# riveSunder/therldaisyworld

Measured on AMD Instinct MI355X. Metric: cell-updates/sec (grid x batch), fused stencil+growth step, higher is better.
Workload: dtype f32

## Files before the change

### therldaisyworld_amd/csrc/dw_api.hip

```cpp
#include <hip/hip_runtime.h>

#include <cmath>
#include <cstdarg>
#include <cstdio>
#include <cstdlib>
#include <cstring>
#include <memory>
#include <new>
#include <optional>
#include <type_traits>
#include <vector>

#include "../../include/daisyworld_hip.h"
#include "dw_kernels.hpp"
#include "dw_host_util.hpp"
#include "dw_plan.hpp"
#include "dw_series.hpp"
#include "dw_episode_staging.hpp"

using namespace dw;

static thread_local char g_err[512] = "";

static int fail(int code, const char* fmt, ...) {
// ... 31 lines not shown
struct PinnedMem {
    static int alloc(void** p, size_t n) { return hipHostMalloc(p, n, hipHostMallocDefault); }
    static int release(void* p) { return hipHostFree(p); }
};
template <class T> using DevBuf = Buf<T, DeviceMem>;
template <class T> using PinnedBuf = Buf<T, PinnedMem>;

struct dw_handle {
    dw_params prm;
    hipStream_t stream = nullptr;
    bool own_stream = false;
    size_t cells = 0;
    DevBuf<plane_t> L16[2];
    DevBuf<plane_t> D16[2];
    int cur = 0;
    DevBuf<double> L64;
    DevBuf<double> D64;
    DevBuf<float> U32L;
    DevBuf<float> U32D;
    UnqKind unq_kind = UNQ_F64;
    UnqOwner unq = OWN_NONE;
    bool have_state = false;
    bool stepped = false;
    double L_last = 0.0;
    bool L_per_world = false;
    bool P_per_world = false;
    DevBuf<int> idx;
    DevBuf<double> st;
    DevBuf<int> action;
    DevBuf<int> action_tmp;
// ... 93 lines not shown

struct SyncOnExit {
    hipStream_t stream;
    bool armed = true;
    explicit SyncOnExit(hipStream_t s) : stream(s) {}
    ~SyncOnExit() { if (armed) (void)hipStreamSynchronize(stream); }
    void disarm() { armed = false; }
};

static int alloc_failed(int rc, const char* what, size_t bytes) {
    (void)hipGetLastError();
    const hipError_t e = static_cast<hipError_t>(rc);
    return fail(e == hipErrorOutOfMemory ? DW_ENOMEM : DW_EHIP, "allocating %s (%zu bytes) failed: %s", what, bytes,
                hipGetErrorString(e));
}
template <class B>
static int reserve(B& buf, const char* what, size_t need, size_t first_size = 0) {
    const int rc = buf.reserve(need, first_size);
    return rc ? alloc_failed(rc, what, need) : DW_OK;
}

static int alloc_group(dw_handle* h, const char* what, std::initializer_list<GroupItem<DeviceMem>> group) {
    static int fail_left = -1;
    if (h->created && fail_left < 0)
        if (const char* e = test_hook("DW_TEST_FAIL_GROUP_ALLOC")) fail_left = std::atoi(e);
    const bool armed = h->created && fail_left > 0;
    if (armed) t_fail_in = (int)group.size();
    const int rc = dw::alloc_group(group);
    if (armed && t_fail_in == 0) --fail_left;
    t_fail_in = 0;
    size_t bytes = 0;
    for (const auto& g : group) bytes += g.bytes;
    return rc ? alloc_failed(rc, what, bytes) : DW_OK;
}

static void release_unquantised(dw_handle* h) {
    if (h->unq != OWN_NONE || !h->U32L.get()) return;
    for (const auto& sn : h->snap)
        if (sn.valid && sn.unq == OWN_PREV) return;
    if (h->cells * 2 * sizeof(float) < ((size_t)1 << 30)) return;
    (void)hipStreamSynchronize(h->stream);
    h->U32L.reset();
    h->U32D.reset();
}

static void drop_unquantised_previous(dw_handle* h) {
    if (h->unq == OWN_PREV) { h->unq = OWN_NONE; h->stepped = false; }
    release_unquantised(h);
}

static int ensure_u32(dw_handle* h) {
    const size_t n = sizeof(float) * h->cells;
    return alloc_group(h, "two float32 planes", {{h->U32L, n}, {h->U32D, n}});
}

static int ensure_f64(dw_handle* h) {
    const size_t n = sizeof(double) * h->cells;
    return alloc_group(h, "two float64 planes", {{h->L64, n}, {h->D64, n}});
}

static int run_episode_impl(dw_handle* h, int32_t nsteps, const double* L_schedule, int policy_mode,
                            const uint8_t* use_table, const int8_t* table, uint32_t threshold_k,
                            uint8_t* world_alive, uint8_t* agent_ok, dw_world_stats* trace = nullptr,
                            dw_temp_stats* temps = nullptr);
static bool episode_kernel_applies(const dw_handle* h);
enum EpisodeForm { EPISODE_STEPWISE, EPISODE_WORKGROUP, EPISODE_WAVE };
static EpisodeForm episode_form(const dw_handle* h);
static EpisodeForm episode_mlp_form(const dw_handle* h, size_t* lds_bytes = nullptr);
static int worlds_per_block(int cells) { return cells <= 256 ? 4 : (cells <= 1024 ? 2 : 1); }
static int observe_into_scratch(dw_handle* h, double L_init, size_t extra_bytes, bool reward_tail = false);

static int ensure_scratch(dw_handle* h, size_t bytes) { return reserve(h->scratch, "scratch", bytes); }

static int ensure_ep_buf(dw_handle* h, size_t bytes) {
    return reserve(h->ep_buf, "the episode staging buffer", bytes, (size_t)4 << 20);
}

struct EpisodeBuffers {
    using R = EpisodeStaging;
    dw_handle* h;
    const EpisodeStaging S;
    unsigned char* img = nullptr;
    std::vector<PhysF32> p32_own;
    std::vector<unsigned char> ut_own;

    EpisodeBuffers(dw_handle* h_, const EpisodeStaging& S_) : h(h_), S(S_) {}
    bool out_direct = false;
    int alloc(bool staged, bool inputs_only = false) {
        if (int rc = ensure_ep_buf(h, S.total)) return rc;
        if (!staged) return DW_OK;
        const size_t image = inputs_only ? S.off[R::WORLD_ALIVE] : S.total;
        if (int rc = reserve(h->ep_pinned, "the page-locked episode staging", image, (size_t)1 << 20)) return rc;
        img = h->ep_pinned.get();
        out_direct = inputs_only;
        return DW_OK;
    }
    template <class T = unsigned char>
    T* dev(R::Region r) const { return S.at<T>(h->ep_buf.get(), r); }
    PhysF32* p32() {
        if (img) return S.at<PhysF32>(img, R::P32);
        p32_own.resize(S.bytes[R::P32] / sizeof(PhysF32));
        return p32_own.data();
    }
    int upload(const double* Ls, size_t n_ls, bool first, const uint8_t* use_table, const int8_t* table) {
        const bool have_table = table && S.bn;
        const size_t ut_bytes = S.bytes[R::USE_TABLE];
        auto to_dev = [&](R::Region r, const void* src, size_t bytes) {
// ... 204 lines not shown
        FixQ fq;
        fq.entries = h->fixq.get();
        fq.counts = reinterpret_cast<unsigned int*>(o.stats + p.batch + 1);
        fq.qcap = h->qcap;
        fq.redo_tiles = h->redo_tiles.get();
        auto tiled = [&](auto TCQ, auto RPT) {
            return with_bool(ex, [&](auto EX) { return launch_tiled<TCQ, RPT, EX>(h, iL, iD, o, fq); });
        };
        if (pl.tcq == 64) return with_int<8, 4, 2>(pl.rpt, [&](auto RPT) { return tiled(int_c<64>{}, RPT); });
        return pl.tcq == 32 ? tiled(int_c<32>{}, int_c<4>{}) : tiled(int_c<16>{}, int_c<2>{});
    }
    HIPCHK(hipGetLastError());
    return DW_OK;
}

static void step_done(dw_handle* h, double L, bool stepped, bool per_world = false, bool per_world_constants = false) {
    h->cur = 1 - h->cur;
    h->sp = 1 - h->sp;
    h->unq = h->unq == OWN_CUR ? OWN_PREV : OWN_NONE;
    h->stepped = stepped;
    h->L_last = L;
    h->L_per_world = per_world;
    h->P_per_world = per_world && per_world_constants;
    release_unquantised(h);
}

static void episode_done(dw_handle* h, double L_last, bool per_world) {
    h->unq = OWN_NONE;
    h->stepped = true;
    h->L_last = per_world ? 0.0 : L_last;
    h->L_per_world = per_world;
    h->P_per_world = per_world;
// ... 312 lines not shown
            });
        });
    } else {
        with_bool(pstats != nullptr, [&](auto STATS) {
            with_fused_layout(pl, [&](auto MODE, auto PACK) {
                hipLaunchKernelGGL((step_stream_fused2<MODE, PACK, STATS>), grid, dim3(256), 0, h->stream, inL, inD, o.L, o.D, g,
                                   P1, P2, o.zero_me, o.zero_n, pstats, thr_hi);
            });
        });
    }
    HIPCHK(hipGetLastError());
    step_done(h, L2, false);
    return DW_OK;
}

static int launch_agents(dw_handle* h, const int* d_action, int act_b, int act_n, bool standalone = false,
                         double* d_reward = nullptr, unsigned char* d_done = nullptr, unsigned char* d_ok = nullptr) {
    const dw_params& p = h->prm;
    if (p.n_agents == 0) return DW_OK;
    NEED(h->have_state, DW_ESTATE, "no state uploaded");
    NEED(h->have_agents, DW_ESTATE, "no agents uploaded (call dw_upload_agents or dw_init_random)");
    NEED(p.collision_mode == 0 || standalone, DW_EINVAL,
         "collision_mode=1: call dw_update_agents, apply the collision pass (it consumes the caller's RNG) to the "
         "downloaded agent states, upload them, then dw_step without actions");
    const int blocks = (p.batch + 63) / 64;
    with_planes(h, h->unq == OWN_CUR, h->cur, [&](auto* L, auto* D) {
        using T = elem_t<decltype(L)>;
        hipLaunchKernelGGL(agents_update<T>, dim3(blocks), dim3(64), 0, h->stream, L, D, h->idx.get(), h->st.get(), d_action,
                           act_b, act_n, p.batch, p.n_agents, p.height, p.width, p.agent_gamma,
                           p.collision_mode == 0 ? 1 : 0, d_reward, d_done, d_ok);
// ... 491 lines not shown
        HIPCHK(hipEventRecord(h->evf0, h->stream));
        int launched = 0;
        while (nsteps - s0 >= 3) {
            const double L1 = L;
            advance();
            const double L2 = L;
            advance();
            int rc = launch_forward_fused2(h, L1, L2);
            if (rc) return rc;
            s0 += 2;
            launched += 1;
        }
        HIPCHK(hipEventRecord(h->evf1, h->stream));
        h->fused_launches = launched;
    }
    for (int s = s0; s < nsteps; ++s) {
        int rc;
        if (use_device_actions) {
            rc = launch_agents(h, h->action.get(), h->prm.batch, h->prm.n_agents);
            if (rc) return rc;
        }
        rc = launch_forward(h, L);
        if (rc) return rc;
        advance();
    }
    *L_io = L;
    return DW_OK;
}

static bool ensemble_pairs(const dw_handle* h) { return h->plan.trace_pairs && h->prm.precision == DW_PRECISION_FAST; }
// ... 13 lines not shown
}

struct PwTable {
    dw_handle* h;
    const PwLayout lay;
    hipEvent_t uploaded = nullptr;
    bool in_flight = false;
    PwTable(dw_handle* h_, const PwLayout& lay_) : h(h_), lay(lay_) {}
    PwTable(const PwTable&) = delete;
    ~PwTable() { if (uploaded) (void)hipEventDestroy(uploaded); }
    unsigned char* img() const { return h->pw_pinned.get(); }
    unsigned char* dev() const { return h->pw_tab.get(); }
    GroupItem<DeviceMem> item() const { return {h->pw_tab, lay.bytes}; }
    int alloc(const char* what, std::initializer_list<GroupItem<DeviceMem>> group) {
        if (int rc = alloc_group(h, what, group)) return rc;
        if (int rc = reserve(h->pw_pinned, "the page-locked image of the per-world constants", lay.bytes)) {
            h->pw_tab.reset();
            return rc;
        }
        HIPCHK(hipEventCreateWithFlags(&uploaded, hipEventDisableTiming));
        return DW_OK;
    }
    int next_chunk(const SeriesSchedule& q, size_t c, const double* Ls, WorldRows& worlds, bool first_bound = false) {
        if (in_flight) HIPCHK(hipEventSynchronize(uploaded));
        fill_chunk(q, c, Ls, worlds, lay, img());
        if (first_bound) worlds.first_bound(Ls, lay.p32(img(), 0), h->unq_kind == UNQ_F64, h->sw.first_slack, lay.fb(img()));
        auto part = [&](size_t off, size_t bytes) { return hipMemcpyAsync(dev() + off, img() + off, bytes, hipMemcpyHostToDevice, h->stream); };
        const size_t singles = q.chunks[c].singles, pairs = q.chunks[c].pairs;
        if (singles) {
            HIPCHK(part(0, sizeof(PhysF32) * singles * lay.B));
            HIPCHK(part(lay.o64, sizeof(PhysF64) * singles * lay.B));
// ... 318 lines not shown
    HIPCHK(hipMemcpyAsync(obs, h->scratch.get(), sizeof(double) * bn * 63, hipMemcpyDeviceToHost, h->stream));
    HIPCHK(hipStreamSynchronize(h->stream));
    return DW_OK;
}

int dw_env_step(dw_handle* h, const int32_t* action, int32_t action_b, int32_t action_n, double L, double* obs,
                double* reward, uint8_t* done) {
    NEED(h, DW_EINVAL, "null handle");
    const dw_params& p = h->prm;
    HIPCHK(hipSetDevice(p.device));
    const size_t bn = (size_t)p.batch * p.n_agents;
    auto up = [](size_t v) { return (v + 255) / 256 * 256; };
    const bool big_obs = sizeof(double) * bn * 63 > ((size_t)512 << 10);
    const size_t o_act = 0, o_obs = up(sizeof(int) * bn), o_rew = o_obs + sizeof(double) * bn * 63;
    const size_t total = up(o_rew + sizeof(double) * bn + bn) + 256;
    if (int rc = reserve(h->pinned, "the page-locked step staging", total)) return rc;
    if (action) {
        NEED(action_b >= 0 && action_n >= 0 && action_b <= p.batch && action_n <= p.n_agents, DW_EINVAL,
             "action block %dx%d exceeds (B,N)=(%d,%d)", action_b, action_n, p.batch, p.n_agents);
        const size_t na = (size_t)action_b * action_n;
        if (na) {
            std::memcpy(h->pinned.get() + o_act, action, sizeof(int) * na);
            HIPCHK(hipMemcpyAsync(h->action_tmp.get(), h->pinned.get() + o_act, sizeof(int) * na, hipMemcpyHostToDevice, h->stream));
        }
        int rc = launch_agents(h, h->action_tmp.get(), action_b, action_n);
        if (rc) return rc;
    }
    int rc = launch_forward(h, L);
    if (rc) return rc;
    if (bn) {
        NEED(h->have_agents, DW_ESTATE, "no agents");
// ... 178 lines not shown
    NEED(n_members == 1 || (member_a && member_b), DW_EINVAL, "several parameter sets need both member maps");
    NEED_SHARED_L(h, "the episode's first observation");
    const size_t wbytes = sizeof(double) * 1808 * (size_t)n_members;
    EpisodeRegions regions;
    regions.rows = K; regions.mlp = true; regions.trace = records; regions.temps = temps != nullptr;
    const EpisodeStaging S(K, (size_t)B, (size_t)N, regions);
    using R = EpisodeStaging;
    const size_t o_ma = S.off[R::MEMBER_A], o_mb = S.off[R::MEMBER_B], o_p32 = S.off[R::P32], o_ls = S.off[R::LS];
    if (temps)
        if (int rc = alloc_group(h, "the temperature reduction", {{h->temp_part, temp_part_bytes(h)}})) return rc;
    if (int erc = ensure_ep_buf(h, S.total)) return erc;
    if (params) {
        if (h->mlp_members != n_members) {
            h->mlp_w.reset();
            h->mlp_members = 0;
            if (int rc = reserve(h->mlp_w, "the parameter sets", wbytes)) return rc;
            h->mlp_members = n_members;
        }
    }
    const double* d_w = h->mlp_w.get();
    const int* d_ma = member_a ? reinterpret_cast<const int*>(h->ep_buf.get() + o_ma) : nullptr;
    const int* d_mb = member_b ? reinterpret_cast<const int*>(h->ep_buf.get() + o_mb) : nullptr;
    double* d_r = S.at<double>(h->ep_buf.get(), R::REWARD);
    unsigned char* d_d = S.at<unsigned char>(h->ep_buf.get(), R::DONE);
    StatsDev* const d_rows = S.at<StatsDev>(h->ep_buf.get(), R::TRACE);
    TempStatsDev* const d_trows = reinterpret_cast<TempStatsDev*>(h->ep_buf.get() + S.temps_off());
    SyncOnExit guard(h->stream);
    if (params) HIPCHK(hipMemcpyAsync(h->mlp_w.get(), params, wbytes, hipMemcpyHostToDevice, h->stream));
    if (member_a) HIPCHK(hipMemcpyAsync(h->ep_buf.get() + o_ma, member_a, sizeof(int) * B, hipMemcpyHostToDevice, h->stream));
    if (member_b) HIPCHK(hipMemcpyAsync(h->ep_buf.get() + o_mb, member_b, sizeof(int) * B, hipMemcpyHostToDevice, h->stream));
    const int Cc = p.height * p.width;
// ... 750 lines not shown
                 g.chunk * 8);
        if (pl.allow_fuse) {
            const size_t n = std::strlen(buf);
            snprintf(buf + n, buflen - n, "; dw_step_n fuses step pairs (step_stream_fused2%s%s",
                     p.precision == DW_PRECISION_EXACT ? "_exact" : "",
                     pl.seam_strips ? "_seam_pw, format buffer accesses" : (pl.fmt_planes ? "_fmt_pw, format buffer accesses" : ""));
            if (pl.seam_strips) {
                const size_t m = std::strlen(buf);
                snprintf(buf + m, buflen - m, ", seam strips: %d x %d columns + %d columns of %d row bands per wave", pl.seam_geom.ncs,
                         kSeamCols, pl.left_geom.cols_per_strip, pl.left_geom.wpr);
            }
            if (pl.row_landing) {
                const size_t m = std::strlen(buf);
                snprintf(buf + m, buflen - m, ", rows land in place: step_stream_fused2_land_seam_pw + _land_left_pw");
            }
            const size_t m = std::strlen(buf);
            snprintf(buf + m, buflen - m, ")");
        }
    } else if (pl.kind == STEP_TILED) {
        const int TR = (256 / pl.tcq) * pl.rpt;
        snprintf(buf, buflen,
                 "step_tiled<TCQ=%d,RPT=%d,%s> tile=%dx%d cells, %zu B LDS/workgroup, %d tiles, grid=%d x 256 threads, "
                 "XCD-chunked",
                 pl.tcq, pl.rpt, prec, TR, pl.tcq * 4, pl.tile_lds, pl.geom.ntiles, pl.geom.chunk * 8);
    } else {
        snprintf(buf, buflen, "step_generic<%s> one thread per cell, grid=(%d,%d) x 256 threads", prec,
                 (p.height * p.width + 255) / 256, p.batch);
    }
    {
        const size_t n = std::strlen(buf);
// ... 92 lines not shown
```

### therldaisyworld_amd/csrc/dw_host_util.hpp

```cpp
#pragma once
#include <cstddef>
#include <initializer_list>

namespace dw {

template <class Policy>
class Block {
public:
    Block() = default;
    Block(const Block&) = delete;
    Block& operator=(const Block&) = delete;
    Block(Block&& o) noexcept : p_(o.p_), bytes_(o.bytes_) { o.p_ = nullptr; o.bytes_ = 0; }
    Block& operator=(Block&& o) noexcept {
        if (this != &o) {
            reset();
            p_ = o.p_; bytes_ = o.bytes_;
            o.p_ = nullptr; o.bytes_ = 0;
        }
        return *this;
    }
    ~Block() { reset(); }

    void* raw() const { return p_; }
    size_t bytes() const { return bytes_; }
// ... 17 lines not shown
        bytes_ = bytes;
        return 0;
    }

private:
    void* p_ = nullptr;
    size_t bytes_ = 0;
};

template <class T, class Policy>
class Buf : public Block<Policy> {
public:
    T* get() const { return static_cast<T*>(this->raw()); }
};

template <class Policy>
struct GroupItem {
    Block<Policy>& owner;
    size_t bytes;
};

template <class Policy>
int alloc_group(std::initializer_list<GroupItem<Policy>> group) {
    bool held = true;
    for (const auto& g : group) held = held && g.owner.bytes() >= g.bytes;
    if (held) return 0;
    for (const auto& g : group) g.owner.reset();
    for (const auto& g : group) {
        if (const int rc = g.owner.take(g.bytes)) {
            for (const auto& r : group) r.owner.reset();
// ... 8 lines not shown
```

### therldaisyworld_amd/csrc/dw_plan.hpp

```cpp
#pragma once
#include <climits>
#include <cmath>
#include <cstddef>
#include <cstdio>
#include <cstdlib>
#include <cstring>

#include "../../include/daisyworld_hip.h"
#include "dw_types.hpp"

namespace dw {

struct Switches {
    bool no_sym = false, no_pack = false, no_fuse = false, no_ring = false, no_fmt_planes = false, no_seam_strips = false,
         no_row_landing = false,
         no_episode_kernel = false,
         no_episode_wave = false, no_agent_fuse = false, no_agent_preapply = false, first_f64 = false,
         first_generic = false, force_rescan = false, test_hooks = false;
    int pack_min_strips = -1, strip_rows = 0, tile_rpt = 0, queue_cap = -1, mismatch_cap = -1, trace_rows = 0, frame_ring = 0;
    double first_slack = -1.0;
    char kernel[16] = {0};
    char text[256] = {0};
};
inline const char* test_hook(const char* name) {
    return std::getenv("DW_TEST_HOOKS") ? std::getenv(name) : nullptr;
}
inline Switches read_switches() {
    Switches w;
    auto note = [&](const char* name, const char* val) {
        const size_t n = std::strlen(w.text);
        snprintf(w.text + n, sizeof(w.text) - n, "%s%s%s%s", n ? " " : "", name, val ? "=" : "", val ? val : "");
    };
    auto flag = [&](const char* name, bool& dst) { if (std::getenv(name)) { dst = true; note(name, nullptr); } };
    auto num = [&](const char* name, int& dst, bool test) {
        if (const char* e = test ? test_hook(name) : std::getenv(name)) { dst = std::atoi(e); note(name, e); }
    };
    w.test_hooks = std::getenv("DW_TEST_HOOKS") != nullptr;
    flag("DW_NO_SYM", w.no_sym); flag("DW_NO_PACK", w.no_pack); flag("DW_NO_FUSE", w.no_fuse); flag("DW_NO_RING", w.no_ring);
    flag("DW_NO_FMT_PLANES", w.no_fmt_planes); flag("DW_NO_SEAM_STRIPS", w.no_seam_strips);
    flag("DW_NO_ROW_LANDING", w.no_row_landing);
    flag("DW_NO_EPISODE_KERNEL", w.no_episode_kernel); flag("DW_NO_EPISODE_WAVE", w.no_episode_wave);
    flag("DW_NO_AGENT_FUSE", w.no_agent_fuse); flag("DW_NO_AGENT_PREAPPLY", w.no_agent_preapply);
    flag("DW_FIRST_STEP_F64", w.first_f64); flag("DW_FIRST_GENERIC", w.first_generic);
    num("DW_PACK_MIN_STRIPS", w.pack_min_strips, false); num("DW_STRIP_ROWS", w.strip_rows, false);
    num("DW_TILE_RPT", w.tile_rpt, false);
    num("DW_TEST_QUEUE_CAP", w.queue_cap, true); num("DW_TEST_MISMATCH_CAP", w.mismatch_cap, true);
    num("DW_TEST_TRACE_ROWS", w.trace_rows, true);
    num("DW_TEST_FRAME_RING", w.frame_ring, true);
    if (test_hook("DW_TEST_FORCE_RESCAN")) { w.force_rescan = true; note("DW_TEST_FORCE_RESCAN", nullptr); }
    if (const char* e = test_hook("DW_TEST_FIRST_SLACK")) { w.first_slack = std::atof(e); note("DW_TEST_FIRST_SLACK", e); }
    if (const char* e = std::getenv("DW_KERNEL")) { snprintf(w.kernel, sizeof(w.kernel), "%s", e); note("DW_KERNEL", e); }
    return w;
}

inline dw_params with_world_params(dw_params p, const dw_world_params& w) {
// ... 230 lines not shown
    auto launch = [](FusedGeom& g, long nstrips) {
        g.nstrips = (int)nstrips;
        g.nwg = (g.nstrips + 3) / 4;
        g.chunk = (g.nwg + 7) / 8;
    };
    *seam = f;
    seam->cols_per_strip = kSeamCols;
    seam->ncs = n_full;
    launch(*seam, (long)f.B * f.nrs * n_full);
    *left = *seam;
    left->cols_per_strip = L;
    left->lpw = L ? L / 4 + 2 : 64;
    left->wpr = 64 / left->lpw;
    launch(*left, L ? (long)f.B * ((f.nrs + left->wpr - 1) / left->wpr) : 0);
    return true;
}

inline StepPlan plan_steps(const dw_params& p, const Switches& sw) {
    StepPlan s;
    s.sym_albedo = albedo_symmetric(p.albedo_bare, p.albedo_light, p.albedo_dark) && !sw.no_sym;
    s.halo = halo_form(p.width);
    const int lpw = p.width / 4, wpr = lpw ? 64 / lpw : 0;
    const bool pack_shape = p.width >= 8 && p.width < 256 && wpr >= 1 && wpr * lpw * 10 >= 64 * 7 && !sw.no_pack;
    const long pack_strips = pack_shape ? (long)((p.batch + wpr - 1) / wpr) * ((p.height + 63) / 64) : 0;
    const bool packable = pack_shape && pack_strips >= (sw.pack_min_strips >= 0 ? sw.pack_min_strips : 512);
    const bool quads = p.precision != DW_PRECISION_F64 && p.width % 4 == 0;
    if (quads && (p.width >= 256 || packable) && std::strcmp(sw.kernel, "tiled") != 0) {
        s.kind = STEP_STREAM;
        s.packed = p.width < 256;
        StripGeom& g = s.sgeom;
// ... 76 lines not shown
```

### therldaisyworld_amd/csrc/dw_step_fused.hpp

```cpp
#pragma once
#include <type_traits>
#include "dw_step_stream.hpp"
#include "dw_types.hpp"

namespace dw {


template <typename TI>
__device__ inline unsigned int exact1_word(const TI* __restrict__ pL, const TI* __restrict__ pD, int H, int W,
                                           int r, int c, const PhysF64& Pa) {
    const int rr = wrap_near2(r, H), cc = wrap_near2(c, W);
    const int ru = rr == 0 ? H - 1 : rr - 1, rd = rr == H - 1 ? 0 : rr + 1;
    const int cl = cc == 0 ? W - 1 : cc - 1, cr = cc == W - 1 ? 0 : cc + 1;
    const int rows[3] = {ru, rr, rd}, cols[3] = {cl, cc, cr};
    unsigned int w1[9];
#pragma unroll
    for (int x = 0; x < 3; ++x)
#pragma unroll
        for (int y = 0; y < 3; ++y) {
            const size_t o = (size_t)rows[x] * W + cols[y];
            w1[x * 3 + y] = (unsigned)(float)pL[o] | ((unsigned)(float)pD[o] << 16);
        }
    const NewCoverF64 s1 = cell_f64_lean(Pa, w1);
    return (unsigned)dw_round3_k(s1.nl) | ((unsigned)dw_round3_k(s1.nd) << 16);
// ... 18 lines not shown
            for (int x = 0; x < 3; ++x)
#pragma unroll
                for (int y = 0; y < 3; ++y) {
                    const size_t o = (size_t)rows[x] * W + cols[y];
                    w1[x * 3 + y] = (unsigned)(float)pL[o] | ((unsigned)(float)pD[o] << 16);
                }
            const NewCoverF64 s1 = cell_f64_lean(Pa, w1);
            w2[a * 3 + e] = (unsigned)dw_round3_k(s1.nl) | ((unsigned)dw_round3_k(s1.nd) << 16);
        }
    const NewCoverF64 s2 = cell_f64_lean(Pb, w2);
    kl = (float)dw_round3_k(s2.nl);
    kd = (float)dw_round3_k(s2.nd);
}

template <int MODE, bool EXACT, bool PACK = false, bool STATS = false, bool SYM = false, typename TI = plane_t,
          typename TO = plane_t, bool TRACE = false, bool FMT = false, int SEAM = kSeamNone, bool LAND = false>
__device__ __forceinline__ void fused2_body(const TI* __restrict__ inL, const TI* __restrict__ inD,
                                            TO* __restrict__ outL, TO* __restrict__ outD, const FusedGeom& G,
                                            const PhysF32& P1_, const PhysF32& P2_, const PhysF64& P64,
                                            const double& La, const double& Lb,
                                            unsigned long long* __restrict__ zero_me, int zero_n,
                                            unsigned int* __restrict__ pstats = nullptr, float thr_hi = 0.f,
                                            StatsDev* __restrict__ trace = nullptr, int trace_rescan = 0) {
    constexpr bool ROT = MODE == kFusedRot, RING = MODE == kFusedRing;
    static_assert(!RING || !PACK, "the ring exchange is written for un-packed worlds");
    static_assert(!TRACE || (!PACK && !STATS && !RING), "the trace form exists for un-packed overlapped / rotating strips");
    static_assert(SEAM == kSeamNone || FMT, "the seam strips exist for the format-access kernel");
    static_assert(!LAND || SEAM != kSeamNone, "rows land in their window slots in the two seam-strip forms");
    static_assert(!FMT || (MODE == kFusedOvl && !EXACT && !PACK && !STATS && !TRACE), "the format-access form exists for the plain float32 kernel on overlapped strips");
    __shared__ float s_edge[RING ? 2 * 4 * 8 : 1];
    __shared__ uint4 s_queue[EXACT ? 4 * kWaveQueueCap * 3 : 1];
    __shared__ unsigned int s_mm[EXACT ? 4 * kMismatchCap : 1];
    const int bid = blockIdx.x;
    const int wg = (bid & 7) * G.chunk + (bid >> 3);
    if (wg >= G.nwg) return;
    const int tid = threadIdx.x, wv = tid >> 6, lane = tid & 63;
    if (wg == 0)
        for (int i = tid; i < zero_n; i += 256) zero_me[i] = 0ull;
    const int s = RING ? wg : __builtin_amdgcn_readfirstlane(wg * 4 + wv);
// ... 52 lines not shown
    const TI* pL = inL + woff;
    const TI* pD = inD + woff;

    dw_i32x4 fmt_inL, fmt_inD, fmt_outL, fmt_outD;
    int fmt_col = 0, fmt_row = 0, fmt_col_b = 0;
    if constexpr (FMT) {
        const unsigned int world_bytes = (unsigned int)(G.H * G.W) * 2u;
        fmt_inL = fmt_plane_rsrc(inL, b, world_bytes, (SEAM == kSeamStrip || LAND) ? kFmtRsrcPairs : kFmtRsrcQuads);
        fmt_inD = fmt_plane_rsrc(inD, b, world_bytes, (SEAM == kSeamStrip || LAND) ? kFmtRsrcPairs : kFmtRsrcQuads);
        fmt_outL = fmt_plane_rsrc(outL, b, world_bytes);
        fmt_outD = fmt_plane_rsrc(outD, b, world_bytes);
        fmt_col = col * 2;
        fmt_col_b = col_b * 2;
        fmt_row = G.W * 2;
    }
    struct RawIn { std::conditional_t<FMT, float4, dw_f16x4> l, d; };
    auto load_raw = [&](int rr) -> RawIn {
        RawIn w;
        if constexpr (SEAM == kSeamLeft) {
            int lr = min(rr + band_dr, r0 + band_dr + band_nr + 1);
            lr = lr < 0 ? lr + G.H : lr;
            lr = lr >= G.H ? lr - G.H : lr;
            if constexpr (LAND) {
                w.l = fmt_load2x2(fmt_inL, fmt_col + lr * fmt_row, fmt_col_b + lr * fmt_row, 0);
                w.d = fmt_load2x2(fmt_inD, fmt_col + lr * fmt_row, fmt_col_b + lr * fmt_row, 0);
                return w;
            }
            w.l = fmt_load4(fmt_inL, fmt_col + lr * fmt_row, 0);
            w.d = fmt_load4(fmt_inD, fmt_col + lr * fmt_row, 0);
            return w;
// ... 51 lines not shown
        }
        ring_par ^= 1;
    };
    unsigned int nq = 0;
#ifndef DW_PIN_CONSTS
#define DW_PIN_CONSTS -1
#endif
    PhysF32 P1 = P1_, P2 = P2_;
    constexpr int PIN = DW_PIN_CONSTS < 0 ? (MODE == kFusedOvl ? 14 : (MODE == kFusedRing ? 8 : 0)) : DW_PIN_CONSTS;
    if constexpr (EXACT && PIN != 0 && !STATS && !PACK) {
        if constexpr ((PIN & 1) != 0) asm volatile("" : "+v"(P1.c0l), "+v"(P2.c0l));
        if constexpr ((PIN & 2) != 0) { asm volatile("" : "+v"(P1.pck)); P2.pck = P1.pck; }
        if constexpr ((PIN & 4) != 0) { asm volatile("" : "+v"(P1.eKb)); P2.eKb = P1.eKb; }
        if constexpr ((PIN & 8) != 0) { asm volatile("" : "+v"(P1.gt)); P2.gt = P1.gt; }
    }
    if constexpr (LAND) { asm volatile("" : "+v"(P1.pck)); P2.pck = P1.pck; }
    constexpr bool CHEAP = STATS && !PACK;
    float st_m1 = 0.f, st_x1 = 0.f;
    unsigned int st_c2 = 0, st_nmm = 0, st_c2w = 0;
    bool st_sure1 = false;
    const unsigned long long writes_mask = CHEAP ? lane_mask(writes) : 0ull;
    const float thr_c2 = EXACT ? thr_hi + 1.0f : thr_hi;
    dw_f32x2 tr_l1 = dw_f32x2(0.f), tr_d1 = dw_f32x2(0.f), tr_l2 = dw_f32x2(0.f), tr_d2 = dw_f32x2(0.f);
    int tr_m1 = 0, tr_m2 = 0;
    float tr_fix_l1 = 0.f, tr_fix_d1 = 0.f, tr_fix_l2 = 0.f, tr_fix_d2 = 0.f;
    float tr_x1 = 0.f, tr_new2 = 0.f, tr_low2 = 0.f;
    auto trace_patch2 = [&](float o, float n) {
        tr_new2 = fmaxf(tr_new2, n);
        if (n < o) tr_low2 = fmaxf(tr_low2, o);
    };
    auto trace_step1 = [&](const float* ol, const float* od, const TieT* tie) {
// ... 273 lines not shown
            } else if constexpr (LAND) {
                to_rows4(make_float4(l1[0], l1[1], l1[2], l1[3]), make_float4(d1[0], d1[1], d1[2], d1[3]), SL[u], SD[u]);
                __builtin_amdgcn_sched_barrier(0);
                landed(std::integral_constant<int, (SEAM == kSeamStrip && do2) ? 2 : 0>{}, IL[(u + 2) % 3], ID[(u + 2) % 3]);
                pin_edge_sums(IL[(u + 2) % 3], ID[(u + 2) % 3]);
            } else {
                to_rows4(make_float4(l1[0], l1[1], l1[2], l1[3]), make_float4(d1[0], d1[1], d1[2], d1[3]), SL[u], SD[u]);
                __builtin_amdgcn_sched_barrier(0);
                to_rows4(widen4(nx.l), widen4(nx.d), IL[(u + 2) % 3], ID[(u + 2) % 3]);
                if (!PACK) pin_edge_sums(IL[(u + 2) % 3], ID[(u + 2) % 3]);
            }
        }
    };
    using Yes = std::true_type;
    using No = std::false_type;
    iter(U1{}, Yes{}, No{}, 1, Yes{}, No{});
    iter(U2{}, Yes{}, No{}, 2, Yes{}, No{});
    iter(U0{}, Yes{}, No{}, 3, Yes{}, No{});
    const int jend = nr + 2;
    const int jloop = TRACE ? jend - 1 : jend;
    int j = 4;
    for (; j + 2 <= jloop; j += 3) {
        iter(U1{}, Yes{}, Yes{}, j, Yes{}, Yes{});
        iter(U2{}, Yes{}, Yes{}, j + 1, Yes{}, Yes{});
        iter(U0{}, Yes{}, Yes{}, j + 2, Yes{}, Yes{});
        if (EXACT && !STATS && __builtin_expect(nq >= (unsigned)flush_at, 0)) sweep_queue();
        if (CHEAP && st_sure1 && st_c2w >= (unsigned int)G.sure_need) { j += 3; break; }
    }
    if constexpr (CHEAP) {
        for (; j + 2 <= jend; j += 3) {
            iter(U1{}, Yes{}, Yes{}, j, No{}, No{});
            iter(U2{}, Yes{}, Yes{}, j + 1, No{}, No{});
            iter(U0{}, Yes{}, Yes{}, j + 2, No{}, No{});
        }
    }
    if (j <= jend) { iter(U1{}, Yes{}, Yes{}, j, Yes{}, No{}); ++j; }
    if (j <= jend) { iter(U2{}, Yes{}, Yes{}, j, Yes{}, No{}); ++j; }
    if constexpr (TRACE) {
        if (j <= jend) { iter(U0{}, Yes{}, Yes{}, j, Yes{}, No{}); ++j; }
    }
    if (j % 3 == 1) iter(U1{}, No{}, Yes{}, j, Yes{}, No{});
    else if (j % 3 == 2) iter(U2{}, No{}, Yes{}, j, Yes{}, No{});
    else iter(U0{}, No{}, Yes{}, j, Yes{}, No{});

    if (EXACT) {
        PhysF64 Pa = P64, Pb = P64;
        Pa.L = La;
        Pb.L = Lb;
        if (RING) {
            wait_row_stores_before_patching();
            __syncthreads();
        }
        sweep_queue();
        if (nmm > (unsigned)G.mcap) redo = true;
        if (RING) {
            wait_row_stores_before_patching();
            __syncthreads();
        }
// ... 250 lines not shown
    const PhysF64 dummy{};
    const double zero = 0.0;
    fused2_body<kFusedOvl, false, false, false, false, plane_t, plane_t, false, true, kSeamStrip, true>(inL, inD, outL, outD, G, P1, P2,
                                                                                                       dummy, zero, zero, zero_me, zero_n);
}
__global__ __launch_bounds__(256) __attribute__((amdgpu_waves_per_eu(DW_FUSED_FAST_WAVES, DW_FUSED_FAST_WAVES)))
void step_stream_fused2_land_left_pw(const plane_t* __restrict__ inL, const plane_t* __restrict__ inD,
                                     plane_t* __restrict__ outL, plane_t* __restrict__ outD, FusedGeom G, PhysF32 P1, PhysF32 P2,
                                     unsigned long long* __restrict__ zero_me, int zero_n) {
    const PhysF64 dummy{};
    const double zero = 0.0;
    fused2_body<kFusedOvl, false, false, false, false, plane_t, plane_t, false, true, kSeamLeft, true>(inL, inD, outL, outD, G, P1, P2,
                                                                                                      dummy, zero, zero, zero_me, zero_n);
}

#ifndef DW_EXACT_PACK_WAVES
#define DW_EXACT_PACK_WAVES 3
#endif
template <int MODE, bool PACK, bool STATS>
constexpr int fused_exact_waves() {
    return (PACK && STATS) || (STATS && MODE == kFusedRing) ? 2 : (PACK ? DW_EXACT_PACK_WAVES : 3);
}
struct FusedExactArgs {
    const plane_t* inL; const plane_t* inD; plane_t* outL; plane_t* outD;
    FusedGeom G;
    PhysF32 P1; PhysLumF32 lum2;
    unsigned long long* zero_me; int zero_n;
    unsigned int* pstats; float thr_hi;
    PhysF64 P64; double La; double Lb;
};
// ... 46 lines not shown
```

Baseline: 837.5 billion.

## Close even step runs with a fused two-step kernel that writes a spare mid plane

```diff
diff --git a/therldaisyworld_amd/csrc/dw_api.hip b/therldaisyworld_amd/csrc/dw_api.hip
--- a/therldaisyworld_amd/csrc/dw_api.hip
+++ b/therldaisyworld_amd/csrc/dw_api.hip
@@ -69,6 +69,9 @@
     DevBuf<plane_t> L16[2];
     DevBuf<plane_t> D16[2];
     int cur = 0;
+    DevBuf<plane_t> spareL, spareD;
+    bool spare_refused = false;
+    int closing_launches = 0;
     DevBuf<double> L64;
     DevBuf<double> D64;
     DevBuf<float> U32L;
@@ -192,21 +195,37 @@
     return fail(e == hipErrorOutOfMemory ? DW_ENOMEM : DW_EHIP, "allocating %s (%zu bytes) failed: %s", what, bytes,
                 hipGetErrorString(e));
 }
+static bool release_spare(dw_handle* h) {
+    if (!h->spareL.get() && !h->spareD.get()) return false;
+    (void)hipStreamSynchronize(h->stream);
+    h->spareL.reset();
+    h->spareD.reset();
+    (void)hipGetLastError();
+    return true;
+}
+static void memory_returned(dw_handle* h) { h->spare_refused = false; }
+
 template <class B>
-static int reserve(B& buf, const char* what, size_t need, size_t first_size = 0) {
-    const int rc = buf.reserve(need, first_size);
+static int reserve(dw_handle* h, B& buf, const char* what, size_t need, size_t first_size = 0) {
+    int rc = buf.reserve(need, first_size);
+    if (rc == (int)hipErrorOutOfMemory && release_spare(h)) rc = buf.reserve(need, first_size);
     return rc ? alloc_failed(rc, what, need) : DW_OK;
 }
 
 static int alloc_group(dw_handle* h, const char* what, std::initializer_list<GroupItem<DeviceMem>> group) {
     static int fail_left = -1;
-    if (h->created && fail_left < 0)
-        if (const char* e = test_hook("DW_TEST_FAIL_GROUP_ALLOC")) fail_left = std::atoi(e);
-    const bool armed = h->created && fail_left > 0;
-    if (armed) t_fail_in = (int)group.size();
-    const int rc = dw::alloc_group(group);
-    if (armed && t_fail_in == 0) --fail_left;
-    t_fail_in = 0;
+    auto attempt = [&]() -> int {
+        if (h->created && fail_left < 0)
+            if (const char* e = test_hook("DW_TEST_FAIL_GROUP_ALLOC")) fail_left = std::atoi(e);
+        const bool armed = h->created && fail_left > 0;
+        if (armed) t_fail_in = (int)group.size();
+        const int r = dw::alloc_group(group);
+        if (armed && t_fail_in == 0) --fail_left;
+        t_fail_in = 0;
+        return r;
+    };
+    int rc = attempt();
+    if (rc == (int)hipErrorOutOfMemory && release_spare(h)) rc = attempt();
     size_t bytes = 0;
     for (const auto& g : group) bytes += g.bytes;
     return rc ? alloc_failed(rc, what, bytes) : DW_OK;
@@ -220,6 +239,7 @@
     (void)hipStreamSynchronize(h->stream);
     h->U32L.reset();
     h->U32D.reset();
+    memory_returned(h);
 }
 
 static void drop_unquantised_previous(dw_handle* h) {
@@ -248,10 +268,10 @@
 static int worlds_per_block(int cells) { return cells <= 256 ? 4 : (cells <= 1024 ? 2 : 1); }
 static int observe_into_scratch(dw_handle* h, double L_init, size_t extra_bytes, bool reward_tail = false);
 
-static int ensure_scratch(dw_handle* h, size_t bytes) { return reserve(h->scratch, "scratch", bytes); }
+static int ensure_scratch(dw_handle* h, size_t bytes) { return reserve(h, h->scratch,"scratch", bytes); }
 
 static int ensure_ep_buf(dw_handle* h, size_t bytes) {
-    return reserve(h->ep_buf, "the episode staging buffer", bytes, (size_t)4 << 20);
+    return reserve(h, h->ep_buf,"the episode staging buffer", bytes, (size_t)4 << 20);
 }
 
 struct EpisodeBuffers {
@@ -268,7 +288,7 @@
         if (int rc = ensure_ep_buf(h, S.total)) return rc;
         if (!staged) return DW_OK;
         const size_t image = inputs_only ? S.off[R::WORLD_ALIVE] : S.total;
-        if (int rc = reserve(h->ep_pinned, "the page-locked episode staging", image, (size_t)1 << 20)) return rc;
+        if (int rc = reserve(h, h->ep_pinned,"the page-locked episode staging", image, (size_t)1 << 20)) return rc;
         img = h->ep_pinned.get();
         out_direct = inputs_only;
         return DW_OK;
@@ -503,8 +523,9 @@
     return DW_OK;
 }
 
-static void step_done(dw_handle* h, double L, bool stepped, bool per_world = false, bool per_world_constants = false) {
-    h->cur = 1 - h->cur;
+static void step_done(dw_handle* h, double L, bool stepped, bool per_world = false, bool per_world_constants = false,
+                      bool cur_flipped = false) {
+    if (!cur_flipped) h->cur = 1 - h->cur;
     h->sp = 1 - h->sp;
     h->unq = h->unq == OWN_CUR ? OWN_PREV : OWN_NONE;
     h->stepped = stepped;
@@ -847,6 +868,37 @@
     return DW_OK;
 }
 
+static bool ensure_spare(dw_handle* h) {
+    const size_t pb = sizeof(plane_t) * h->cells;
+    if (h->spareL.bytes() >= pb && h->spareD.bytes() >= pb) return true;
+    if (h->spare_refused) return false;
+    if (alloc_group(h, "the spare plane pair", {{h->spareL, pb}, {h->spareD, pb}}) != DW_OK) {
+        h->spare_refused = true;
+        return false;
+    }
+    return true;
+}
+
+static int launch_closing_pair(dw_handle* h, double L1, double L2) {
+    const dw_params& p = h->prm;
+    const StepPlan& pl = h->plan;
+    const PhysF32 P1 = derive_f32(p, L1), P2 = derive_f32(p, L2);
+    const StepOut o = step_out(h);
+    const FusedGeom &gs = pl.seam_geom, &gl = pl.left_geom;
+    const plane_t *inL = h->L16[h->cur].get(), *inD = h->D16[h->cur].get();
+    plane_t *midL = h->spareL.get(), *midD = h->spareD.get();
+    hipLaunchKernelGGL(step_stream_fused2_close_seam_pw, dim3((unsigned)gs.chunk * 8u), dim3(256), 0, h->stream, inL, inD, o.L,
+                       o.D, midL, midD, gs, P1, P2, o.zero_me, o.zero_n, o.stats);
+    if (gl.nstrips)
+        hipLaunchKernelGGL(step_stream_fused2_close_left_pw, dim3((unsigned)gl.chunk * 8u), dim3(256), 0, h->stream, inL, inD,
+                           o.L, o.D, midL, midD, gl, P1, P2, o.zero_me, 0, o.stats);
+    HIPCHK(hipGetLastError());
+    rotate_spare(h->L16, h->D16, h->spareL, h->spareD, h->cur);
+    step_done(h, L2, true, false, false, true);
+    h->closing_launches += 1;
+    return DW_OK;
+}
+
 static int launch_agents(dw_handle* h, const int* d_action, int act_b, int act_n, bool standalone = false,
                          double* d_reward = nullptr, unsigned char* d_done = nullptr, unsigned char* d_ok = nullptr) {
     const dw_params& p = h->prm;
@@ -1368,6 +1420,15 @@
         HIPCHK(hipEventRecord(h->evf1, h->stream));
         h->fused_launches = launched;
     }
+    if (!use_device_actions && h->have_state &&
+        closing_pair_applies(h->plan, h->sw, h->prm.precision, nsteps - s0, cur_quantised(h)) && ensure_spare(h)) {
+        const double L1 = L;
+        advance();
+        const double L2 = L;
+        advance();
+        if (int rc = launch_closing_pair(h, L1, L2)) return rc;
+        s0 += 2;
+    }
     for (int s = s0; s < nsteps; ++s) {
         int rc;
         if (use_device_actions) {
@@ -1411,7 +1472,7 @@
     GroupItem<DeviceMem> item() const { return {h->pw_tab, lay.bytes}; }
     int alloc(const char* what, std::initializer_list<GroupItem<DeviceMem>> group) {
         if (int rc = alloc_group(h, what, group)) return rc;
-        if (int rc = reserve(h->pw_pinned, "the page-locked image of the per-world constants", lay.bytes)) {
+        if (int rc = reserve(h, h->pw_pinned,"the page-locked image of the per-world constants", lay.bytes)) {
             h->pw_tab.reset();
             return rc;
         }
@@ -1760,7 +1821,7 @@
     const bool big_obs = sizeof(double) * bn * 63 > ((size_t)512 << 10);
     const size_t o_act = 0, o_obs = up(sizeof(int) * bn), o_rew = o_obs + sizeof(double) * bn * 63;
     const size_t total = up(o_rew + sizeof(double) * bn + bn) + 256;
-    if (int rc = reserve(h->pinned, "the page-locked step staging", total)) return rc;
+    if (int rc = reserve(h, h->pinned,"the page-locked step staging", total)) return rc;
     if (action) {
         NEED(action_b >= 0 && action_n >= 0 && action_b <= p.batch && action_n <= p.n_agents, DW_EINVAL,
              "action block %dx%d exceeds (B,N)=(%d,%d)", action_b, action_n, p.batch, p.n_agents);
@@ -1969,7 +2030,7 @@
         if (h->mlp_members != n_members) {
             h->mlp_w.reset();
             h->mlp_members = 0;
-            if (int rc = reserve(h->mlp_w, "the parameter sets", wbytes)) return rc;
+            if (int rc = reserve(h, h->mlp_w,"the parameter sets", wbytes)) return rc;
             h->mlp_members = n_members;
         }
     }
@@ -2750,6 +2811,11 @@
                 const size_t m = std::strlen(buf);
                 snprintf(buf + m, buflen - m, ", rows land in place: step_stream_fused2_land_seam_pw + _land_left_pw");
             }
+            if (closing_pair_applies(pl, h->sw, p.precision, 2, true)) {
+                const size_t m = std::strlen(buf);
+                snprintf(buf + m, buflen - m, ", even runs close on step_stream_fused2_close_seam_pw + _close_left_pw: %d closing launches%s",
+                         h->closing_launches, h->spare_refused ? " (no room for the spare planes: two single steps)" : "");
+            }
             const size_t m = std::strlen(buf);
             snprintf(buf + m, buflen - m, ")");
         }
diff --git a/therldaisyworld_amd/csrc/dw_host_util.hpp b/therldaisyworld_amd/csrc/dw_host_util.hpp
--- a/therldaisyworld_amd/csrc/dw_host_util.hpp
+++ b/therldaisyworld_amd/csrc/dw_host_util.hpp
@@ -55,6 +55,16 @@
     T* get() const { return static_cast<T*>(this->raw()); }
 };
 
+template <class B>
+void rotate_spare(B (&L)[2], B (&D)[2], B& spareL, B& spareD, int& cur) {
+    B tL(static_cast<B&&>(L[cur])), tD(static_cast<B&&>(D[cur]));
+    L[cur] = static_cast<B&&>(spareL);
+    D[cur] = static_cast<B&&>(spareD);
+    spareL = static_cast<B&&>(tL);
+    spareD = static_cast<B&&>(tD);
+    cur = 1 - cur;
+}
+
 template <class Policy>
 struct GroupItem {
     Block<Policy>& owner;
diff --git a/therldaisyworld_amd/csrc/dw_plan.hpp b/therldaisyworld_amd/csrc/dw_plan.hpp
--- a/therldaisyworld_amd/csrc/dw_plan.hpp
+++ b/therldaisyworld_amd/csrc/dw_plan.hpp
@@ -13,7 +13,7 @@
 
 struct Switches {
     bool no_sym = false, no_pack = false, no_fuse = false, no_ring = false, no_fmt_planes = false, no_seam_strips = false,
-         no_row_landing = false,
+         no_row_landing = false, no_closing_pair = false,
          no_episode_kernel = false,
          no_episode_wave = false, no_agent_fuse = false, no_agent_preapply = false, first_f64 = false,
          first_generic = false, force_rescan = false, test_hooks = false;
@@ -38,7 +38,7 @@
     w.test_hooks = std::getenv("DW_TEST_HOOKS") != nullptr;
     flag("DW_NO_SYM", w.no_sym); flag("DW_NO_PACK", w.no_pack); flag("DW_NO_FUSE", w.no_fuse); flag("DW_NO_RING", w.no_ring);
     flag("DW_NO_FMT_PLANES", w.no_fmt_planes); flag("DW_NO_SEAM_STRIPS", w.no_seam_strips);
-    flag("DW_NO_ROW_LANDING", w.no_row_landing);
+    flag("DW_NO_ROW_LANDING", w.no_row_landing); flag("DW_NO_CLOSING_PAIR", w.no_closing_pair);
     flag("DW_NO_EPISODE_KERNEL", w.no_episode_kernel); flag("DW_NO_EPISODE_WAVE", w.no_episode_wave);
     flag("DW_NO_AGENT_FUSE", w.no_agent_fuse); flag("DW_NO_AGENT_PREAPPLY", w.no_agent_preapply);
     flag("DW_FIRST_STEP_F64", w.first_f64); flag("DW_FIRST_GENERIC", w.first_generic);
@@ -299,6 +299,12 @@
     left->wpr = 64 / left->lpw;
     launch(*left, L ? (long)f.B * ((f.nrs + left->wpr - 1) / left->wpr) : 0);
     return true;
+}
+
+constexpr int kCloseMaxRows = 4096;
+inline bool closing_pair_applies(const StepPlan& pl, const Switches& sw, int precision, long remaining, bool quantised) {
+    return remaining == 2 && quantised && precision == DW_PRECISION_FAST && pl.kind == STEP_STREAM && pl.allow_fuse &&
+           pl.row_landing && !sw.no_closing_pair && pl.seam_geom.SR <= kCloseMaxRows;
 }
 
 inline StepPlan plan_steps(const dw_params& p, const Switches& sw) {
diff --git a/therldaisyworld_amd/csrc/dw_step_fused.hpp b/therldaisyworld_amd/csrc/dw_step_fused.hpp
--- a/therldaisyworld_amd/csrc/dw_step_fused.hpp
+++ b/therldaisyworld_amd/csrc/dw_step_fused.hpp
@@ -56,15 +56,18 @@
 }
 
 template <int MODE, bool EXACT, bool PACK = false, bool STATS = false, bool SYM = false, typename TI = plane_t,
-          typename TO = plane_t, bool TRACE = false, bool FMT = false, int SEAM = kSeamNone, bool LAND = false>
+          typename TO = plane_t, bool TRACE = false, bool FMT = false, int SEAM = kSeamNone, bool LAND = false,
+          bool CLOSE = false>
 __device__ __forceinline__ void fused2_body(const TI* __restrict__ inL, const TI* __restrict__ inD,
                                             TO* __restrict__ outL, TO* __restrict__ outD, const FusedGeom& G,
                                             const PhysF32& P1_, const PhysF32& P2_, const PhysF64& P64,
                                             const double& La, const double& Lb,
                                             unsigned long long* __restrict__ zero_me, int zero_n,
                                             unsigned int* __restrict__ pstats = nullptr, float thr_hi = 0.f,
-                                            StatsDev* __restrict__ trace = nullptr, int trace_rescan = 0) {
+                                            StatsDev* __restrict__ trace = nullptr, int trace_rescan = 0,
+                                            TO* __restrict__ midL = nullptr, TO* __restrict__ midD = nullptr) {
     constexpr bool ROT = MODE == kFusedRot, RING = MODE == kFusedRing;
+    static_assert(!CLOSE || LAND, "the closing form exists for the row-landing seam-strip kernels");
     static_assert(!RING || !PACK, "the ring exchange is written for un-packed worlds");
     static_assert(!TRACE || (!PACK && !STATS && !RING), "the trace form exists for un-packed overlapped / rotating strips");
     static_assert(SEAM == kSeamNone || FMT, "the seam strips exist for the format-access kernel");
@@ -147,6 +150,12 @@
         fmt_col_b = col_b * 2;
         fmt_row = G.W * 2;
     }
+    dw_i32x4 fmt_midL, fmt_midD;
+    if constexpr (CLOSE) {
+        const unsigned int world_bytes = (unsigned int)(G.H * G.W) * 2u;
+        fmt_midL = fmt_plane_rsrc(midL, b, world_bytes);
+        fmt_midD = fmt_plane_rsrc(midD, b, world_bytes);
+    }
     struct RawIn { std::conditional_t<FMT, float4, dw_f16x4> l, d; };
     auto load_raw = [&](int rr) -> RawIn {
         RawIn w;
@@ -228,7 +237,7 @@
         if constexpr ((PIN & 4) != 0) { asm volatile("" : "+v"(P1.eKb)); P2.eKb = P1.eKb; }
         if constexpr ((PIN & 8) != 0) { asm volatile("" : "+v"(P1.gt)); P2.gt = P1.gt; }
     }
-    if constexpr (LAND) { asm volatile("" : "+v"(P1.pck)); P2.pck = P1.pck; }
+    if constexpr (LAND && !(CLOSE && SEAM == kSeamLeft)) { asm volatile("" : "+v"(P1.pck)); P2.pck = P1.pck; }
     constexpr bool CHEAP = STATS && !PACK;
     float st_m1 = 0.f, st_x1 = 0.f;
     unsigned int st_c2 = 0, st_nmm = 0, st_c2w = 0;
@@ -532,6 +541,110 @@
     };
     using Yes = std::true_type;
     using No = std::false_type;
+    if constexpr (CLOSE) {
+        __shared__ float s_red[3 * 256];
+        __shared__ unsigned int s_tot[4 * 4];
+        float* const red = s_red + tid;
+        unsigned int* const tot = s_tot + 4 * __builtin_amdgcn_readfirstlane(wv);
+        red[0] = 0.f; red[256] = 0.f; red[512] = 0.f;
+        if (lane < 3) tot[lane] = 0u;
+        auto reduce_step2 = [&](const float* ol, const float* od) {
+            const dw_f32x2 tl = dw_f32x2{ol[0], ol[1]} + dw_f32x2{ol[2], ol[3]}, td = dw_f32x2{od[0], od[1]} + dw_f32x2{od[2], od[3]};
+            const float m = fmaxf(fmaxf(fmaxf(ol[0], ol[1]), fmaxf(ol[2], ol[3])), fmaxf(fmaxf(od[0], od[1]), fmaxf(od[2], od[3])));
+            (void)__hip_atomic_fetch_add(red, tl.x, __ATOMIC_RELAXED, __HIP_MEMORY_SCOPE_WORKGROUP);
+            (void)__hip_atomic_fetch_add(red, tl.y, __ATOMIC_RELAXED, __HIP_MEMORY_SCOPE_WORKGROUP);
+            (void)__hip_atomic_fetch_add(red + 256, td.x, __ATOMIC_RELAXED, __HIP_MEMORY_SCOPE_WORKGROUP);
+            (void)__hip_atomic_fetch_add(red + 256, td.y, __ATOMIC_RELAXED, __HIP_MEMORY_SCOPE_WORKGROUP);
+            (void)__hip_atomic_fetch_max(reinterpret_cast<int*>(red + 512), __float_as_int(m), __ATOMIC_RELAXED, __HIP_MEMORY_SCOPE_WORKGROUP);
+        };
+        auto iter_close = [&](auto U, auto D1, auto D2, int j, auto MINE) {
+            constexpr int u = decltype(U)::value;
+            constexpr bool do1 = decltype(D1)::value, do2 = decltype(D2)::value, mine = decltype(MINE)::value;
+            UpSums4 up1;
+            if constexpr (do1) {
+                up1 = up_sums4(IL[(u + 2) % 3], IL[(u + 1) % 3], ID[(u + 2) % 3], ID[(u + 1) % 3]);
+                asm volatile("" : "+v"(up1.xl[0]), "+v"(up1.xl[1]), "+v"(up1.cl[0]), "+v"(up1.cl[1]),
+                                  "+v"(up1.xd[0]), "+v"(up1.xd[1]), "+v"(up1.cd[0]), "+v"(up1.cd[1]));
+                __builtin_amdgcn_sched_barrier(0);
+                land_row(r0 + j, IL[(u + 2) % 3], ID[(u + 2) % 3]);
+            }
+            __builtin_amdgcn_sched_barrier(0);
+            float l1[4], d1[4], l2[4], d2[4];
+            TieT tie2[4];
+            if constexpr (do2)
+                row_cells(P2, SL[u], SL[(u + 1) % 3], SL[(u + 2) % 3], SD[u], SD[(u + 1) % 3], SD[(u + 2) % 3], l2, d2, tie2,
+                          use2, nullptr);
+            if constexpr (do1) cells4_up(P1, up1, IL[u], ID[u], l1, d1);
+            if constexpr (do2) {
+                if constexpr (SEAM == kSeamLeft) {
+                    if (j - 4 < band_nr) reduce_step2(l2, d2);
+                    if (writes && j - 4 < band_nr) {
+                        const int voff = fmt_col + (r0 + band_dr + j - 4) * fmt_row;
+                        fmt_store4(fmt_outL, voff, 0, make_float4(l2[0], l2[1], l2[2], l2[3]));
+                        fmt_store4(fmt_outD, voff, 0, make_float4(d2[0], d2[1], d2[2], d2[3]));
+                    }
+                } else {
+                    reduce_step2(l2, d2);
+                    if (writes) {
+                        fmt_store4(fmt_outL, fmt_col, (r0 + j - 4) * fmt_row, make_float4(l2[0], l2[1], l2[2], l2[3]));
+                        fmt_store4(fmt_outD, fmt_col, (r0 + j - 4) * fmt_row, make_float4(d2[0], d2[1], d2[2], d2[3]));
+                    }
+                }
+            }
+            if constexpr (do1) {
+                if constexpr (SEAM == kSeamLeft) {
+                    if (writes && j >= 2 && j - 2 < band_nr) {
+                        const int voff = fmt_col + (r0 + band_dr + j - 2) * fmt_row;
+                        fmt_store4(fmt_midL, voff, 0, make_float4(l1[0], l1[1], l1[2], l1[3]));
+                        fmt_store4(fmt_midD, voff, 0, make_float4(d1[0], d1[1], d1[2], d1[3]));
+                    }
+                } else if (mine || (j >= 2 && j <= nr + 1)) {
+                    if (writes) {
+                        fmt_store4(fmt_midL, fmt_col, (r0 + j - 2) * fmt_row, make_float4(l1[0], l1[1], l1[2], l1[3]));
+                        fmt_store4(fmt_midD, fmt_col, (r0 + j - 2) * fmt_row, make_float4(d1[0], d1[1], d1[2], d1[3]));
+                    }
+                }
+                to_rows4(make_float4(l1[0], l1[1], l1[2], l1[3]), make_float4(d1[0], d1[1], d1[2], d1[3]), SL[u], SD[u]);
+                __builtin_amdgcn_sched_barrier(0);
+                constexpr int younger = SEAM == kSeamStrip ? (do2 ? 2 : 0) + (mine ? 2 : 0) : 0;
+                landed(std::integral_constant<int, younger>{}, IL[(u + 2) % 3], ID[(u + 2) % 3]);
+                pin_edge_sums(IL[(u + 2) % 3], ID[(u + 2) % 3]);
+            }
+        };
+        iter_close(U1{}, Yes{}, No{}, 1, No{});
+        iter_close(U2{}, Yes{}, No{}, 2, Yes{});
+        iter_close(U0{}, Yes{}, No{}, 3, No{});
+        const int jend = nr + 2;
+        int j = 4;
+        for (; j + 2 <= jend - 1; j += 3) {
+            iter_close(U1{}, Yes{}, Yes{}, j, Yes{});
+            iter_close(U2{}, Yes{}, Yes{}, j + 1, Yes{});
+            iter_close(U0{}, Yes{}, Yes{}, j + 2, Yes{});
+        }
+        if (j <= jend) { iter_close(U1{}, Yes{}, Yes{}, j, No{}); ++j; }
+        if (j <= jend) { iter_close(U2{}, Yes{}, Yes{}, j, No{}); ++j; }
+        if (j <= jend) { iter_close(U0{}, Yes{}, Yes{}, j, No{}); ++j; }
+        if (j % 3 == 1) iter_close(U1{}, No{}, Yes{}, j, No{});
+        else if (j % 3 == 2) iter_close(U2{}, No{}, Yes{}, j, No{});
+        else iter_close(U0{}, No{}, Yes{}, j, No{});
+        __builtin_amdgcn_fence(__ATOMIC_RELEASE, "wavefront");
+        __builtin_amdgcn_wave_barrier();
+        if (writes) {
+            atomicAdd(&tot[0], (unsigned int)red[0]);
+            atomicAdd(&tot[1], (unsigned int)red[256]);
+            atomicMax(&tot[2], (unsigned int)red[512]);
+        }
+        __builtin_amdgcn_fence(__ATOMIC_RELEASE, "wavefront");
+        __builtin_amdgcn_wave_barrier();
+        __builtin_amdgcn_fence(__ATOMIC_ACQUIRE, "wavefront");
+        if (__builtin_amdgcn_mbcnt_hi(~0u, __builtin_amdgcn_mbcnt_lo(~0u, 0u)) == 0u) {
+            StatsDev* const t2 = trace + b;
+            atomicMax(&t2->max_k, tot[2]);
+            atomicAdd(&t2->sum_l, (unsigned long long)tot[0]);
+            atomicAdd(&t2->sum_d, (unsigned long long)tot[1]);
+        }
+    }
+    if constexpr (!CLOSE) {
     iter(U1{}, Yes{}, No{}, 1, Yes{}, No{});
     iter(U2{}, Yes{}, No{}, 2, Yes{}, No{});
     iter(U0{}, Yes{}, No{}, 3, Yes{}, No{});
@@ -560,6 +673,7 @@
     if (j % 3 == 1) iter(U1{}, No{}, Yes{}, j, Yes{}, No{});
     else if (j % 3 == 2) iter(U2{}, No{}, Yes{}, j, Yes{}, No{});
     else iter(U0{}, No{}, Yes{}, j, Yes{}, No{});
+    }
 
     if (EXACT) {
         PhysF64 Pa = P64, Pb = P64;
@@ -840,6 +954,27 @@
                                                                                                       dummy, zero, zero, zero_me, zero_n);
 }
 
+__global__ __launch_bounds__(256) __attribute__((amdgpu_waves_per_eu(DW_FUSED_FAST_WAVES, DW_FUSED_FAST_WAVES)))
+void step_stream_fused2_close_seam_pw(const plane_t* __restrict__ inL, const plane_t* __restrict__ inD,
+                                      plane_t* __restrict__ outL, plane_t* __restrict__ outD, plane_t* __restrict__ midL,
+                                      plane_t* __restrict__ midD, FusedGeom G, PhysF32 P1, PhysF32 P2,
+                                      unsigned long long* __restrict__ zero_me, int zero_n, StatsDev* __restrict__ stats) {
+    const PhysF64 dummy{};
+    const double zero = 0.0;
+    fused2_body<kFusedOvl, false, false, false, false, plane_t, plane_t, false, true, kSeamStrip, true, true>(
+        inL, inD, outL, outD, G, P1, P2, dummy, zero, zero, zero_me, zero_n, nullptr, 0.f, stats, 0, midL, midD);
+}
+__global__ __launch_bounds__(256) __attribute__((amdgpu_waves_per_eu(DW_FUSED_FAST_WAVES, DW_FUSED_FAST_WAVES)))
+void step_stream_fused2_close_left_pw(const plane_t* __restrict__ inL, const plane_t* __restrict__ inD,
+                                      plane_t* __restrict__ outL, plane_t* __restrict__ outD, plane_t* __restrict__ midL,
+                                      plane_t* __restrict__ midD, FusedGeom G, PhysF32 P1, PhysF32 P2,
+                                      unsigned long long* __restrict__ zero_me, int zero_n, StatsDev* __restrict__ stats) {
+    const PhysF64 dummy{};
+    const double zero = 0.0;
+    fused2_body<kFusedOvl, false, false, false, false, plane_t, plane_t, false, true, kSeamLeft, true, true>(
+        inL, inD, outL, outD, G, P1, P2, dummy, zero, zero, zero_me, zero_n, nullptr, 0.f, stats, 0, midL, midD);
+}
+
 #ifndef DW_EXACT_PACK_WAVES
 #define DW_EXACT_PACK_WAVES 3
 #endif
```

New measurement: 828.1 billion. 1.1% lower.
